# PPWangyc/video-spike

Hardware: AMD Instinct MI355X
Metric: clips/sec (16-frame 224x224) train step (higher is better)
Workload: dtype bf16; 1 GPU; C2 ViT-Tiny/16 16x224x224 -> 128 neurons, encoder+head fwd+bwd+AdamW; model=vmae_tiny, global_batch=128, clips_per_gpu=128, seq_len=1568, parallelism=dp1

## Files before the change

video-spike_amd/csrc/attention.hip:

```cpp
#include <math.h>
#include <stdlib.h>

#include <type_traits>

#include "common.h"

namespace vs {

constexpr float kLog2e = 1.4426950408889634f;
constexpr float kLn2 = 0.6931471805599453f;

__global__ __launch_bounds__(256) void attn_fwd_f32_kernel(const float* __restrict__ qkv, int64_t ldq,
                                                           float* __restrict__ o, int64_t ldo, float* __restrict__ lse,
                                                           int N, int H, float scale) {
  __shared__ float sK[64][68];
  __shared__ float sV[64][68];
  const int tid = threadIdx.x, sub = tid & 3;
  const int qi = blockIdx.x * 64 + (tid >> 2);
  const int h = blockIdx.y, b = blockIdx.z, D = H * 64;
  const int64_t row0 = (int64_t)b * N;
  const float* Qp = qkv + row0 * ldq + h * 64;
  const float* Kp = Qp + D;
  const float* Vp = Qp + 2 * D;
  float q[16], acc[16];
// ... 171 lines not shown
    for (int d = 0; d < 16; ++d) dqkv[(row0 + qi) * ldd + h * 64 + sub * 16 + d] = dq[d] * scale;
  }
}

template <typename T>
__global__ __launch_bounds__(256) void attn_delta_kernel(const T* __restrict__ o, int64_t ldo, const T* __restrict__ dout,
                                                         int64_t lddo, float* __restrict__ delta, int64_t rows, int N,
                                                         int H) {
  const int lane = threadIdx.x & 63;
  const int64_t w = blockIdx.x * 4 + (threadIdx.x >> 6);
  if (w >= rows * H) return;
  const int64_t row = w / H;
  const int h = (int)(w % H);
  float v = Elem<T>::load(o + row * ldo + h * 64 + lane) * Elem<T>::load(dout + row * lddo + h * 64 + lane);
  v = wave_sum(v);
  if (lane == 0) {
    const int64_t b = row / N, n = row % N;
    delta[(b * H + h) * N + n] = v;
  }
}

__device__ __forceinline__ int swz_row(int r) { return (r >> 1) & 7; }
__device__ __forceinline__ int swz_half(int r) { return ((r >> 1) & 1) << 2; }

__device__ __forceinline__ int off_rowswz(int r, int c) { return r * 128 + (((c >> 3) ^ swz_row(r)) << 4) + (c & 7) * 2; }
__device__ __forceinline__ int off_halfswz(int r, int c) { return r * 128 + (((c >> 3) ^ swz_half(r)) << 4) + (c & 7) * 2; }

__device__ __forceinline__ bf16x8 tr_pair(const char* lds, int off0, int off1) {
  short4v t0 = __builtin_amdgcn_ds_read_tr16_b64_v4i16((VS_LDS short4v*)(lds + off0));
  short4v t1 = __builtin_amdgcn_ds_read_tr16_b64_v4i16((VS_LDS short4v*)(lds + off1));
  typedef __attribute__((ext_vector_type(8))) short short8v;
  short8v s = {t0[0], t0[1], t0[2], t0[3], t1[0], t1[1], t1[2], t1[3]};
  return __builtin_bit_cast(bf16x8, s);
}

typedef __attribute__((ext_vector_type(8))) float f32x8;
__device__ __forceinline__ bf16x8 pack8(const f32x16& a, int base) {
  const f32x8 v = {a[base], a[base + 1], a[base + 2], a[base + 3], a[base + 4], a[base + 5], a[base + 6], a[base + 7]};
  return __builtin_convertvector(v, bf16x8);
}
__device__ __forceinline__ bf16x8 pack8f(const float* a) {
  const f32x8 v = {a[0], a[1], a[2], a[3], a[4], a[5], a[6], a[7]};
  return __builtin_convertvector(v, bf16x8);
}

__device__ __forceinline__ uint2 pack4(float a, float b, float c, float d) {
  uint2 u;
  u.x = (uint32_t)f2bf(a) | ((uint32_t)f2bf(b) << 16);
  u.y = (uint32_t)f2bf(c) | ((uint32_t)f2bf(d) << 16);
  return u;
}

constexpr float kRescaleThr = 8.0f;
constexpr float kRefBand = 32.0f;
#ifndef VS_FWD_TOPBAR
#define VS_FWD_TOPBAR 0
#endif

__device__ __forceinline__ float max3f(float a, float b, float c) {
  float r;
  asm volatile("v_max3_f32 %0, %1, %2, %3" : "=v"(r) : "v"(a), "v"(b), "v"(c));
  return r;
}
__device__ __forceinline__ float max16(const f32x16& x) {
  const float a = max3f(x[0], x[1], x[2]), b = max3f(x[3], x[4], x[5]), c = max3f(x[6], x[7], x[8]);
  const float d = max3f(x[9], x[10], x[11]), e = max3f(x[12], x[13], x[14]);
// ... 85 lines not shown
  bf16x8 qf[4];
#pragma unroll
  for (int s = 0; s < 4; ++s) {
    const int qr = qi < N ? qi : N - 1;
    const bf16x8 q = *(const bf16x8*)(Qp + (int64_t)qr * ldq + 16 * s + 8 * hh);
    f32x8 v;
#pragma unroll
    for (int j = 0; j < 8; ++j) v[j] = (float)q[j] * c;
    qf[s] = __builtin_convertvector(v, bf16x8);
  }
  const bf16x8 sel = rowsum_selector(lane);
  f32x16 oacc[2], zero16;
  f32x4 lacc;
  float m_run, l_half;

  const int q4 = (lane & 15) >> 2, p4 = (lane & 3) * 4, g16 = ((lane >> 4) & 1) * 16;
  int kbase[4];
  {
    const int key = lane & 31;
#pragma unroll
    for (int s = 0; s < 4; ++s) kbase[s] = key * 128 + (((2 * s + hh) ^ swz_row(key)) << 4);
  }
  int vbase[2];
  {
    const int k0 = 4 * hh + q4;
#pragma unroll
    for (int dt = 0; dt < 2; ++dt) vbase[dt] = TILE + off_halfswz(k0, dt * 32 + g16 + p4);
  }
  const int prow0 = wid * 16 + (lane >> 3), ppos = lane & 7;
  const uint32_t gk0 = (uint32_t)(prow0 * 2 * ldq + ((ppos ^ swz_row(prow0)) << 4));
  const uint32_t gk1 = (uint32_t)((prow0 + 8) * 2 * ldq + ((ppos ^ swz_row(prow0 + 8)) << 4));
  const uint32_t gv0 = (uint32_t)(prow0 * 2 * ldq + ((ppos ^ swz_half(prow0)) << 4));
  const uint32_t gv1 = (uint32_t)((prow0 + 8) * 2 * ldq + ((ppos ^ swz_half(prow0 + 8)) << 4));
  const int64_t tile_bytes = 64 * 2 * ldq, vdelta = 2 * (int64_t)D;
  auto load_tile = [&](int kt, char* buf) {
    const char* kb = (const char*)Kp + kt * tile_bytes;
    const char* vb = kb + vdelta;
    char* dk = buf + wid * 2048;
    char* dv = buf + TILE + wid * 2048;
    if ((kt + 1) * 64 <= N) {
      glds16_asm_so(kb, gk0, dk);
      glds16_asm_so(kb, gk1, dk + 1024);
      glds16_asm_so(vb, gv0, dv);
      glds16_asm_so(vb, gv1, dv + 1024);
    } else {
      const int r0 = kt * 64 + prow0, r1 = r0 + 8;
      const uint32_t c0 = (uint32_t)((r0 < N ? r0 : N - 1) - kt * 64) * (uint32_t)(2 * ldq);
      const uint32_t c1 = (uint32_t)((r1 < N ? r1 : N - 1) - kt * 64) * (uint32_t)(2 * ldq);
      glds16_asm_so(kb, c0 + ((ppos ^ swz_row(prow0)) << 4), dk);
      glds16_asm_so(kb, c1 + ((ppos ^ swz_row(prow0 + 8)) << 4), dk + 1024);
      glds16_asm_so(vb, c0 + ((ppos ^ swz_half(prow0)) << 4), dv);
      glds16_asm_so(vb, c1 + ((ppos ^ swz_half(prow0 + 8)) << 4), dv + 1024);
    }
  };
  struct KFrag {
    bf16x8 k[4];
  };
  struct VFrag {
    bf16x8 v[4];
  };
  auto kread = [&](const char* base, int kb) {
    KFrag f;
#pragma unroll
    for (int s = 0; s < 4; ++s) f.k[s] = *(const bf16x8*)(base + kb * 4096 + kbase[s]);
    return f;
  };
  auto vread = [&](const char* base, int kb) {
    VFrag f;
#pragma unroll
    for (int s = 0; s < 2; ++s)
#pragma unroll
      for (int dt = 0; dt < 2; ++dt) {
        const char* vb = base + kb * 4096 + s * 2048;
        f.v[2 * s + dt] = tr_pair(vb, vbase[dt], vbase[dt] + 1024);
      }
    return f;
  };
  auto pv = [&](const VFrag& f, const bf16x8& pa, const bf16x8& pb) {
#pragma unroll
    for (int s = 0; s < 2; ++s)
#pragma unroll
      for (int dt = 0; dt < 2; ++dt)
        oacc[dt] = mfma32p(f.v[2 * s + dt], s == 0 ? pa : pb, oacc[dt]);
  };

  auto softmax_m = [&](auto safec, auto maskc, f32x16& acc, int key0, bool first_blk, bf16x8& pa, bf16x8& pb) {
// ... 279 lines not shown
  if (tid == 0) redo_flag = 0;

  bf16x8 qf[2][2];
#pragma unroll
  for (int qt = 0; qt < 2; ++qt) {
    const int qi = q0w + qt * 16 + c, qr = qi < N ? qi : N - 1;
#pragma unroll
    for (int dc = 0; dc < 2; ++dc) {
      const bf16x8 q = *(const bf16x8*)(Qp + (int64_t)qr * ldq + dc * 32 + 8 * g);
      f32x8 v;
#pragma unroll
      for (int j = 0; j < 8; ++j) v[j] = (float)q[j] * scale_log2;
      qf[qt][dc] = __builtin_convertvector(v, bf16x8);
    }
  }
  const bf16x8 ones = __builtin_convertvector((f32x8){1.f, 1.f, 1.f, 1.f, 1.f, 1.f, 1.f, 1.f}, bf16x8);
  f32x4 oacc[4][2], lacc[2];
  const f32x4 zero4 = {0.f, 0.f, 0.f, 0.f};
  float m_run[2], l_half[2];

  int kbase[2], vbase[4];
#pragma unroll
  for (int dc = 0; dc < 2; ++dc) kbase[dc] = c * 128 + (((dc * 4 + g) ^ swz_row(c)) << 4);
  {
    const int r = 4 * g + (c >> 2), sw = swz_v16(r);
#pragma unroll
    for (int dt = 0; dt < 4; ++dt) vbase[dt] = TILE + r * 128 + (((dt * 2 + ((c & 3) >> 1)) ^ sw) << 4) + (c & 1) * 8;
  }
  const int prow0 = wid * 16 + (lane >> 3), ppos = lane & 7;
  const uint32_t gk0 = (uint32_t)(prow0 * 2 * ldq + ((ppos ^ swz_row(prow0)) << 4));
  const uint32_t gk1 = (uint32_t)((prow0 + 8) * 2 * ldq + ((ppos ^ swz_row(prow0 + 8)) << 4));
  const uint32_t gv0 = (uint32_t)(prow0 * 2 * ldq + ((ppos ^ swz_v16(prow0)) << 4));
  const uint32_t gv1 = (uint32_t)((prow0 + 8) * 2 * ldq + ((ppos ^ swz_v16(prow0 + 8)) << 4));
  const int64_t tile_bytes = 64 * 2 * ldq, vdelta = 2 * (int64_t)D;
  auto load_tile = [&](int kt, char* buf) {
    const char* kb = (const char*)Kp + kt * tile_bytes;
    const char* vb = kb + vdelta;
    char* dk = buf + wid * 2048;
    char* dv = buf + TILE + wid * 2048;
    if ((kt + 1) * 64 <= N) {
      glds16_asm_so(kb, gk0, dk);
      glds16_asm_so(kb, gk1, dk + 1024);
      glds16_asm_so(vb, gv0, dv);
      glds16_asm_so(vb, gv1, dv + 1024);
    } else {
      const int r0 = kt * 64 + prow0, r1 = r0 + 8;
      const uint32_t c0 = (uint32_t)((r0 < N ? r0 : N - 1) - kt * 64) * (uint32_t)(2 * ldq);
      const uint32_t c1 = (uint32_t)((r1 < N ? r1 : N - 1) - kt * 64) * (uint32_t)(2 * ldq);
      glds16_asm_so(kb, c0 + ((ppos ^ swz_row(prow0)) << 4), dk);
      glds16_asm_so(kb, c1 + ((ppos ^ swz_row(prow0 + 8)) << 4), dk + 1024);
      glds16_asm_so(vb, c0 + ((ppos ^ swz_v16(prow0)) << 4), dv);
      glds16_asm_so(vb, c1 + ((ppos ^ swz_v16(prow0 + 8)) << 4), dv + 1024);
    }
  };
  struct KFrag {
    bf16x8 k[2][2];
  };
  struct VFrag {
    bf16x8 v[4];
  };
  struct SAcc {
    f32x4 s[2][2];
  };
  auto kread = [&](const char* base, int kb) {
    KFrag f;
#pragma unroll
    for (int ks = 0; ks < 2; ++ks)
#pragma unroll
      for (int dc = 0; dc < 2; ++dc) f.k[ks][dc] = *(const bf16x8*)(base + kb * 4096 + ks * 2048 + kbase[dc]);
    return f;
  };
  auto vread = [&](const char* base, int kb) {
    VFrag f;
#pragma unroll
    for (int dt = 0; dt < 4; ++dt) f.v[dt] = tr_pair(base + kb * 4096, vbase[dt], vbase[dt] + 2048);
    return f;
  };
  auto qk_first = [&](const KFrag& f, SAcc& a) { a.s[0][0] = mfma16(f.k[0][0], qf[0][0], zero4); };
  auto qk_rest = [&](const KFrag& f, SAcc& a) {
    a.s[0][1] = mfma16(f.k[0][0], qf[1][0], zero4);
    a.s[1][0] = mfma16(f.k[1][0], qf[0][0], zero4);
    a.s[1][1] = mfma16(f.k[1][0], qf[1][0], zero4);
#pragma unroll
    for (int ks = 0; ks < 2; ++ks)
#pragma unroll
      for (int qt = 0; qt < 2; ++qt) a.s[ks][qt] = mfma16(f.k[ks][1], qf[qt][1], a.s[ks][qt]);
// ... 223 lines not shown
    nlse2[w] = -INFINITY;
    ndel[w] = 0.f;
  }
}

__device__ __forceinline__ int swz_rt(int r) {
  const int u = (r >> 1) & 7;
  return ((u & 1) << 2) | (u >> 1);
}
__device__ __forceinline__ int off_rtswz(int r, int c) { return r * 128 + (((c >> 3) ^ swz_rt(r)) << 4) + (c & 7) * 2; }

constexpr int kBwdQT = 64 * 128;
constexpr int kBwdStage = 2 * kBwdQT + 512;

__device__ __forceinline__ void attn_bwd_dkdv_body(char* __restrict__ stg0, char* __restrict__ stg1, int blk,
                                                   const bf16_t* __restrict__ qkv, int64_t ldq,
                                                   const bf16_t* __restrict__ dout, int64_t lddo,
                                                   const float* __restrict__ nlse2, const float* __restrict__ ndel,
                                                   bf16_t* __restrict__ dqkv, int64_t ldd, int N, int H, int Npad,
                                                   float scale) {
  constexpr int QT = kBwdQT;
  const int tid = threadIdx.x, lane = tid & 63, wid = __builtin_amdgcn_readfirstlane(tid >> 6), hh = lane >> 5;
  const int nb128 = (N + 127) / 128, kb = blk % nb128;
  const int h = (blk / nb128) % H, b = blk / nb128 / H, D = H * 64;
  const int64_t row0 = (int64_t)b * N;
  const bf16_t* Qp = qkv + row0 * ldq + h * 64;
  const bf16_t* Kp = Qp + D;
  const bf16_t* Vp = Qp + 2 * D;
  const bf16_t* Dp = dout + row0 * lddo + h * 64;
  const float* NL = nlse2 + ((int64_t)b * H + h) * Npad;
  const float* ND = ndel + ((int64_t)b * H + h) * Npad;
  const int ki = kb * 128 + wid * 32 + (lane & 31);
  const float c2 = scale * kLog2e;

  bf16x8 kf[4], vf[4];
  {
    const int kr = ki < N ? ki : N - 1;
#pragma unroll
    for (int s = 0; s < 4; ++s) {
      const bf16x8 k = *(const bf16x8*)(Kp + (int64_t)kr * ldq + 16 * s + 8 * hh);
      f32x8 v;
#pragma unroll
      for (int j = 0; j < 8; ++j) v[j] = (float)k[j] * c2;
      kf[s] = __builtin_convertvector(v, bf16x8);
      vf[s] = *(const bf16x8*)(Vp + (int64_t)kr * ldq + 16 * s + 8 * hh);
    }
  }
  f32x16 dkacc[2], dvacc[2];
#pragma unroll
  for (int r = 0; r < 16; ++r) {
    dkacc[0][r] = 0.f;
    dkacc[1][r] = 0.f;
    dvacc[0][r] = 0.f;
    dvacc[1][r] = 0.f;
  }

  const int prow = wid * 16 + (lane >> 3), ppos = lane & 7;
  const uint32_t cq0 = (uint32_t)((ppos ^ swz_rt(prow)) << 4), cq1 = (uint32_t)((ppos ^ swz_rt(prow + 8)) << 4);
  const uint32_t gq0 = (uint32_t)(prow * 2 * ldq) + cq0, gq1 = (uint32_t)((prow + 8) * 2 * ldq) + cq1;
  const uint32_t gd0 = (uint32_t)(prow * 2 * lddo) + cq0, gd1 = (uint32_t)((prow + 8) * 2 * lddo) + cq1;
  auto load_stage = [&](int it, char* dst) {
    const int q0 = it * 64;
    const char* qs = (const char*)(Qp + (int64_t)q0 * ldq);
    const char* ds = (const char*)(Dp + (int64_t)q0 * lddo);
    char* dq_ = dst + wid * 2048;
    char* dd_ = dst + QT + wid * 2048;
    if (q0 + 64 <= N) {
      glds16_asm_so(qs, gq0, dq_);
      glds16_asm_so(qs, gq1, dq_ + 1024);
// ... 42 lines not shown
    for (int s = 0; s < 4; ++s)
      acc = mfma32p(*(const bf16x8*)(sQ + sub * 4096 + roff[s]), kf[s], acc);
#pragma unroll
    for (int s2 = 0; s2 < 2; ++s2) {
      float p[8], ds[8];
#pragma unroll
      for (int r = 0; r < 8; ++r) {
        p[r] = __builtin_amdgcn_exp2f(acc[8 * s2 + r]);
        ds[r] = p[r] * dpa[8 * s2 + r];
      }
      const bf16x8 pb = pack8f(p), db = pack8f(ds);
#pragma unroll
      for (int dt = 0; dt < 2; ++dt) {
        const int o0 = sub * 4096 + s2 * 2048 + toff[dt][0], o1 = sub * 4096 + s2 * 2048 + toff[dt][1];
        dvacc[dt] = mfma32p(tr_pair(sD, o0, o1), pb, dvacc[dt]);
      }
#pragma unroll
      for (int dt = 0; dt < 2; ++dt) {
        const int o0 = sub * 4096 + s2 * 2048 + toff[dt][0], o1 = sub * 4096 + s2 * 2048 + toff[dt][1];
        dkacc[dt] = mfma32p(tr_pair(sQ, o0, o1), db, dkacc[dt]);
      }
    }
    __builtin_amdgcn_sched_barrier(0);
  };

  const int nit = (N + 63) / 64;
  load_stage(0, stg0);
  auto iter = [&](int it, auto bufc) {
    constexpr int BUF = decltype(bufc)::value;
    asm volatile("s_waitcnt vmcnt(0)" ::: "memory");
    __syncthreads();
    if (it + 1 < nit && !((VS_ATTN_DIAG & 2) && it >= 1)) load_stage(it + 1, BUF ? stg0 : stg1);
    const char* st = BUF ? stg1 : stg0;
    slice(st, 0);
    __builtin_amdgcn_sched_barrier(0);
    if (it * 64 + 32 < N) slice(st, 1);
    __builtin_amdgcn_sched_barrier(0);
  };
  for (int it = 0; it < nit; it += 2) {
    iter(it, IC<0>{});
    if (it + 1 < nit) iter(it + 1, IC<1>{});
  }

  if (ki < N) {
    bf16_t* krow = dqkv + (row0 + ki) * ldd + D + h * 64;
    bf16_t* vrow = krow + D;
#pragma unroll
    for (int dt = 0; dt < 2; ++dt)
#pragma unroll
      for (int g = 0; g < 4; ++g) {
        const int d = dt * 32 + 8 * g + 4 * hh;
        *(uint2*)(krow + d) = pack4(dkacc[dt][4 * g] * scale, dkacc[dt][4 * g + 1] * scale,
                                    dkacc[dt][4 * g + 2] * scale, dkacc[dt][4 * g + 3] * scale);
        *(uint2*)(vrow + d) = pack4(dvacc[dt][4 * g], dvacc[dt][4 * g + 1], dvacc[dt][4 * g + 2], dvacc[dt][4 * g + 3]);
      }
  }
}

__device__ __forceinline__ void attn_bwd_dq_body(char* __restrict__ kv0, char* __restrict__ kv1, int blk,
                                                 const bf16_t* __restrict__ qkv, int64_t ldq,
                                                 const bf16_t* __restrict__ dout, int64_t lddo,
                                                 const float* __restrict__ nlse2, const float* __restrict__ ndel,
                                                 bf16_t* __restrict__ dqkv, int64_t ldd, int N, int H, int Npad,
                                                 float scale) {
  constexpr int TILE = 64 * 128;
  const int tid = threadIdx.x, lane = tid & 63, wid = __builtin_amdgcn_readfirstlane(tid >> 6), hh = lane >> 5;
  const int nb128 = (N + 127) / 128, qb = blk % nb128;
  const int h = (blk / nb128) % H, b = blk / nb128 / H, D = H * 64;
  const int64_t row0 = (int64_t)b * N;
  const bf16_t* Qp = qkv + row0 * ldq + h * 64;
  const bf16_t* Kp = Qp + D;
  const bf16_t* Dp = dout + row0 * lddo + h * 64;
  const int qi = qb * 128 + wid * 32 + (lane & 31);
  const float c2 = scale * kLog2e;

  bf16x8 qf[4], df[4];
  {
    const int qr = qi < N ? qi : N - 1;
#pragma unroll
    for (int s = 0; s < 4; ++s) {
      const bf16x8 q = *(const bf16x8*)(Qp + (int64_t)qr * ldq + 16 * s + 8 * hh);
      f32x8 v;
#pragma unroll
      for (int j = 0; j < 8; ++j) v[j] = (float)q[j] * c2;
      qf[s] = __builtin_convertvector(v, bf16x8);
      df[s] = *(const bf16x8*)(Dp + (int64_t)qr * lddo + 16 * s + 8 * hh);
    }
  }
  f32x16 sinit, dinit, dqacc[2];
  {
    const int64_t w = ((int64_t)b * H + h) * Npad + qi;
    const float nl = qi < N ? nlse2[w] : -INFINITY;
    const float nd = qi < N ? ndel[w] : 0.f;
#pragma unroll
    for (int r = 0; r < 16; ++r) {
      sinit[r] = nl;
      dinit[r] = nd;
      dqacc[0][r] = 0.f;
      dqacc[1][r] = 0.f;
    }
  }

  int roff[4];
  {
    const int key = lane & 31;
#pragma unroll
    for (int s = 0; s < 4; ++s) roff[s] = key * 128 + (((2 * s + hh) ^ swz_rt(key)) << 4);
  }
  const int q4 = (lane & 15) >> 2, p4 = (lane & 3) * 4, g16 = ((lane >> 4) & 1) * 16, kt0 = 4 * hh + q4;
  int toff[2][2];
// ... 36 lines not shown
      const bf16x8 ka = *(const bf16x8*)(sK + kb * 4096 + roff[s]);
      const bf16x8 va = *(const bf16x8*)(sV + kb * 4096 + roff[s]);
      sacc = mfma32p(ka, qf[s], sacc);
      dpacc = mfma32p(va, df[s], dpacc);
    }
    if (key0 + 32 > N) {
#pragma unroll
      for (int r = 0; r < 16; ++r)
        if (key0 + (r & 3) + 8 * (r >> 2) + 4 * hh >= N) sacc[r] = -INFINITY;
    }
#pragma unroll
    for (int s2 = 0; s2 < 2; ++s2) {
      float ds[8];
#pragma unroll
      for (int r = 0; r < 8; ++r) ds[r] = __builtin_amdgcn_exp2f(sacc[8 * s2 + r]) * dpacc[8 * s2 + r];
      const bf16x8 db = pack8f(ds);
#pragma unroll
      for (int dt = 0; dt < 2; ++dt) {
        const int o = kb * 4096 + s2 * 2048;
        const bf16x8 ka = tr_pair(sK, o + toff[dt][0], o + toff[dt][1]);
        dqacc[dt] = mfma32p(ka, db, dqacc[dt]);
      }
    }
  };

  const int nkt = (N + 63) / 64;
  load_tile(0, kv0);
  auto iter = [&](int kt, auto bufc) {
    constexpr int BUF = decltype(bufc)::value;
    asm volatile("s_waitcnt vmcnt(0)" ::: "memory");
    __syncthreads();
    if (kt + 1 < nkt && !((VS_ATTN_DIAG & 2) && kt >= 1)) load_tile(kt + 1, BUF ? kv0 : kv1);
    const char* cur = BUF ? kv1 : kv0;
    sub(cur, 0, kt * 64);
    if (kt * 64 + 32 < N) sub(cur, 1, kt * 64 + 32);
  };
  for (int kt = 0; kt < nkt; kt += 2) {
    iter(kt, IC<0>{});
    if (kt + 1 < nkt) iter(kt + 1, IC<1>{});
  }
  if (qi < N) {
    bf16_t* qrow = dqkv + (row0 + qi) * ldd + h * 64;
#pragma unroll
    for (int dt = 0; dt < 2; ++dt)
#pragma unroll
      for (int g = 0; g < 4; ++g) {
        const int d = dt * 32 + 8 * g + 4 * hh;
        *(uint2*)(qrow + d) = pack4(dqacc[dt][4 * g] * scale, dqacc[dt][4 * g + 1] * scale,
                                    dqacc[dt][4 * g + 2] * scale, dqacc[dt][4 * g + 3] * scale);
      }
  }
}

__device__ __forceinline__ void attn_bwd_dkdv_pp(char* __restrict__ stg0, char* __restrict__ stg1, int blk,
                                                 const bf16_t* __restrict__ qkv, int64_t ldq,
                                                 const bf16_t* __restrict__ dout, int64_t lddo,
                                                 const float* __restrict__ nlse2, const float* __restrict__ ndel,
                                                 bf16_t* __restrict__ dqkv, int64_t ldd, int N, int H, int Npad,
                                                 float scale) {
  constexpr int QT = kBwdQT;
  const int tid = threadIdx.x, lane = tid & 63, hh = lane >> 5;
  const int wid = __builtin_amdgcn_readfirstlane(tid >> 6);
  const int nb128 = (N + 127) / 128, kb = blk % nb128;
  const int h = (blk / nb128) % H, b = blk / nb128 / H, D = H * 64;
  const int64_t row0 = (int64_t)b * N;
  const bf16_t* Qp = qkv + row0 * ldq + h * 64;
  const bf16_t* Kp = Qp + D;
  const bf16_t* Vp = Qp + 2 * D;
  const bf16_t* Dp = dout + row0 * lddo + h * 64;
  const float* NL = nlse2 + ((int64_t)b * H + h) * Npad;
  const float* ND = ndel + ((int64_t)b * H + h) * Npad;
  const int ki = kb * 128 + wid * 32 + (lane & 31);
  const float c2 = scale * kLog2e;

  bf16x8 kf[4], vf[4];
  {
    const int kr = ki < N ? ki : N - 1;
#pragma unroll
    for (int s = 0; s < 4; ++s) {
      const bf16x8 k = *(const bf16x8*)(Kp + (int64_t)kr * ldq + 16 * s + 8 * hh);
      f32x8 v;
#pragma unroll
      for (int j = 0; j < 8; ++j) v[j] = (float)k[j] * c2;
      kf[s] = __builtin_convertvector(v, bf16x8);
      vf[s] = *(const bf16x8*)(Vp + (int64_t)kr * ldq + 16 * s + 8 * hh);
    }
  }
  f32x16 dkacc[2], dvacc[2];
#pragma unroll
  for (int r = 0; r < 16; ++r) {
    dkacc[0][r] = 0.f;
    dkacc[1][r] = 0.f;
    dvacc[0][r] = 0.f;
    dvacc[1][r] = 0.f;
  }
  auto load_stage = [&](int it, char* dst) {
    const int prow = wid * 16 + (lane >> 3), ppos = lane & 7;
    const uint32_t cq0 = (uint32_t)((ppos ^ swz_rt(prow)) << 4), cq1 = (uint32_t)((ppos ^ swz_rt(prow + 8)) << 4);
    const int q0 = it * 64;
    int r0 = prow, r1 = prow + 8;
    if (q0 + 64 > N) {
      r0 = q0 + r0 < N ? r0 : N - 1 - q0;
      r1 = q0 + r1 < N ? r1 : N - 1 - q0;
    }
    const char* qs = (const char*)(Qp + (int64_t)q0 * ldq);
    const char* ds = (const char*)(Dp + (int64_t)q0 * lddo);
    glds16_asm_so(qs, (uint32_t)r0 * (uint32_t)(2 * ldq) + cq0, dst + wid * 2048);
    glds16_asm_so(qs, (uint32_t)r1 * (uint32_t)(2 * ldq) + cq1, dst + wid * 2048 + 1024);
    glds16_asm_so(ds, (uint32_t)r0 * (uint32_t)(2 * lddo) + cq0, dst + QT + wid * 2048);
// ... 67 lines not shown
    rowc(sE, 0, xa);
    mma_p(fa, pa, dvacc);
#pragma unroll
    for (int s = 0; s < 4; ++s) xa = mfma32p(fb[s], vf[s], xa);
    __builtin_amdgcn_sched_barrier(0);
    tr4(sD, 1, fa);
    rows4(sD, 1, fb);
    __builtin_amdgcn_sched_barrier(0);
#pragma unroll
    for (int r = 0; r < 16; ++r) pb[r] = __builtin_amdgcn_exp2f(xb[r]);
    rowc(sE, 1, xb);
    mma_p(fa, pb, dvacc);
#pragma unroll
    for (int s = 0; s < 4; ++s) xb = mfma32p(fb[s], vf[s], xb);
    __builtin_amdgcn_sched_barrier(0);
    tr4(sQ, 0, fa);
    tr4(sQ, 1, fb);
    __builtin_amdgcn_sched_barrier(0);
#pragma unroll
    for (int r = 0; r < 16; ++r) pa[r] *= xa[r];
    mma_p(fa, pa, dkacc);
#pragma unroll
    for (int r = 0; r < 16; ++r) pb[r] *= xb[r];
    mma_p(fb, pb, dkacc);
    __builtin_amdgcn_sched_barrier(0);
  };
  const int nit = (N + 63) / 64;
  load_stage(0, stg0);
  auto iter = [&](int it, auto bufc) {
    constexpr int BUF = decltype(bufc)::value;
    asm volatile("s_waitcnt vmcnt(0)" ::: "memory");
    __syncthreads();
    if (it + 1 < nit) load_stage(it + 1, BUF ? stg0 : stg1);
    slice(BUF ? stg1 : stg0);
  };
  for (int it = 0; it < nit; it += 2) {
    iter(it, IC<0>{});
    if (it + 1 < nit) iter(it + 1, IC<1>{});
  }
  if (ki < N) {
    bf16_t* krow = dqkv + (row0 + ki) * ldd + D + h * 64;
    bf16_t* vrow = krow + D;
#pragma unroll
    for (int dt = 0; dt < 2; ++dt)
#pragma unroll
      for (int g = 0; g < 4; ++g) {
        const int d = dt * 32 + 8 * g + 4 * hh;
        *(uint2*)(krow + d) = pack4(dkacc[dt][4 * g] * scale, dkacc[dt][4 * g + 1] * scale,
                                    dkacc[dt][4 * g + 2] * scale, dkacc[dt][4 * g + 3] * scale);
        *(uint2*)(vrow + d) = pack4(dvacc[dt][4 * g], dvacc[dt][4 * g + 1], dvacc[dt][4 * g + 2], dvacc[dt][4 * g + 3]);
      }
  }
}

__device__ __forceinline__ void attn_bwd_dq_pp(char* __restrict__ kv0, char* __restrict__ kv1, int blk,
                                               const bf16_t* __restrict__ qkv, int64_t ldq,
                                               const bf16_t* __restrict__ dout, int64_t lddo,
                                               const float* __restrict__ nlse2, const float* __restrict__ ndel,
                                               bf16_t* __restrict__ dqkv, int64_t ldd, int N, int H, int Npad,
                                               float scale) {
  constexpr int TILE = 64 * 128;
  const int tid = threadIdx.x, lane = tid & 63, hh = lane >> 5;
  const int wid = __builtin_amdgcn_readfirstlane(tid >> 6);
  const int nb128 = (N + 127) / 128, qb = blk % nb128;
  const int h = (blk / nb128) % H, b = blk / nb128 / H, D = H * 64;
  const int64_t row0 = (int64_t)b * N;
  const bf16_t* Qp = qkv + row0 * ldq + h * 64;
  const bf16_t* Kp = Qp + D;
  const bf16_t* Dp = dout + row0 * lddo + h * 64;
  const int qi = qb * 128 + wid * 32 + (lane & 31);
  const float c2 = scale * kLog2e;
  bf16x8 qf[4], df[4];
  {
    const int qr = qi < N ? qi : N - 1;
#pragma unroll
    for (int s = 0; s < 4; ++s) {
      const bf16x8 q = *(const bf16x8*)(Qp + (int64_t)qr * ldq + 16 * s + 8 * hh);
      f32x8 v;
#pragma unroll
      for (int j = 0; j < 8; ++j) v[j] = (float)q[j] * c2;
      qf[s] = __builtin_convertvector(v, bf16x8);
      df[s] = *(const bf16x8*)(Dp + (int64_t)qr * lddo + 16 * s + 8 * hh);
    }
  }
  f32x16 sinit, dinit, dqacc[2];
  {
    const int64_t w = ((int64_t)b * H + h) * Npad + qi;
    const float nl = qi < N ? nlse2[w] : -INFINITY;
    const float nd = qi < N ? ndel[w] : 0.f;
#pragma unroll
    for (int r = 0; r < 16; ++r) {
      sinit[r] = nl;
      dinit[r] = nd;
      dqacc[0][r] = 0.f;
      dqacc[1][r] = 0.f;
    }
  }
  int roff[4];
  {
    const int key = lane & 31;
#pragma unroll
    for (int s = 0; s < 4; ++s) roff[s] = key * 128 + (((2 * s + hh) ^ swz_rt(key)) << 4);
  }
  const int q4 = (lane & 15) >> 2, p4 = (lane & 3) * 4, g16 = ((lane >> 4) & 1) * 16, kt0 = 4 * hh + q4;
  int toff[2][2];
#pragma unroll
// ... 58 lines not shown
      kb_[s] = *(const bf16x8*)(sK + 4096 + roff[s]);
      vb[s] = *(const bf16x8*)(sV + 4096 + roff[s]);
    }
    __builtin_amdgcn_sched_barrier(0);
#pragma unroll
    for (int s = 0; s < 4; ++s) {
      sa = mfma32p(ka[s], qf[s], s == 0 ? sinit : sa);
      da = mfma32p(va[s], df[s], s == 0 ? dinit : da);
    }
#pragma unroll
    for (int s = 0; s < 4; ++s) {
      sb = mfma32p(kb_[s], qf[s], s == 0 ? sinit : sb);
      db = mfma32p(vb[s], df[s], s == 0 ? dinit : db);
    }
    __builtin_amdgcn_sched_barrier(0);
    ktr4(sK, 0, ka);
    ktr4(sK, 1, kb_);
    __builtin_amdgcn_sched_barrier(0);
    if (key0 + 64 > N) {
      mask(sa, key0);
      mask(sb, key0 + 32);
    }
    dq_mma(ka, sa, da);
    dq_mma(kb_, sb, db);
    __builtin_amdgcn_sched_barrier(0);
  };
  const int nkt = (N + 63) / 64;
  load_tile(0, kv0);
  auto iter = [&](int kt, auto bufc) {
    constexpr int BUF = decltype(bufc)::value;
    asm volatile("s_waitcnt vmcnt(0)" ::: "memory");
    __syncthreads();
    if (kt + 1 < nkt) load_tile(kt + 1, BUF ? kv0 : kv1);
    tile(BUF ? kv1 : kv0, kt * 64);
  };
  for (int kt = 0; kt < nkt; kt += 2) {
    iter(kt, IC<0>{});
    if (kt + 1 < nkt) iter(kt + 1, IC<1>{});
  }
  if (qi < N) {
    bf16_t* qrow = dqkv + (row0 + qi) * ldd + h * 64;
#pragma unroll
    for (int dt = 0; dt < 2; ++dt)
#pragma unroll
      for (int g = 0; g < 4; ++g) {
        const int d = dt * 32 + 8 * g + 4 * hh;
        *(uint2*)(qrow + d) = pack4(dqacc[dt][4 * g] * scale, dqacc[dt][4 * g + 1] * scale,
                                    dqacc[dt][4 * g + 2] * scale, dqacc[dt][4 * g + 3] * scale);
      }
  }
}

template <int WPS, bool PKV, bool PQ>
__global__ __launch_bounds__(256, WPS) void attn_bwd_bf16_pp_kernel(const bf16_t* __restrict__ qkv, int64_t ldq,
                                                                    const bf16_t* __restrict__ dout, int64_t lddo,
                                                                    const float* __restrict__ nlse2,
                                                                    const float* __restrict__ ndel,
                                                                    bf16_t* __restrict__ dqkv, int64_t ldd, int N,
                                                                    int H, int Npad, float scale, int nblk, int skip) {
  __shared__ __attribute__((aligned(16))) char st0[kBwdStage];
  __shared__ __attribute__((aligned(16))) char st1[kBwdStage];
  const int id = blockIdx.x;
  if (skip & (id < nblk ? 1 : 2)) return;
  if (id < nblk) {
    if constexpr (PKV)
      attn_bwd_dkdv_pp(st0, st1, xcd_remap(id, nblk), qkv, ldq, dout, lddo, nlse2, ndel, dqkv, ldd, N, H, Npad, scale);
    else
// ... 17 lines not shown
  __shared__ __attribute__((aligned(16))) char st0[kBwdStage];
  __shared__ __attribute__((aligned(16))) char st1[kBwdStage];
  const int id = blockIdx.x;
  if (skip & (id < nblk ? 1 : 2)) return;
  if (id < nblk)
    attn_bwd_dkdv_body(st0, st1, xcd_remap(id, nblk), qkv, ldq, dout, lddo, nlse2, ndel, dqkv, ldd, N, H, Npad, scale);
  else
    attn_bwd_dq_body(st0, st1, xcd_remap(id - nblk, nblk), qkv, ldq, dout, lddo, nlse2, ndel, dqkv, ldd, N, H, Npad,
                     scale);
}

}

using namespace vs;

static int attn_check(int64_t B, int64_t N, int64_t H, int64_t Dh) {
  VS_REQUIRE(Dh == 64, "vs_attn: head dim must be 64");
  VS_REQUIRE(B > 0 && N > 0 && H > 0, "vs_attn: empty problem");
  VS_REQUIRE(B <= 65535 && H <= 65535 && N < (1 << 30), "vs_attn: extents out of range");
  return VS_OK;
}

extern "C" int vs_attn_fwd(int32_t dtype, int64_t B, int64_t N, int64_t H, int64_t Dh, const void* qkv, int64_t ld_qkv,
                           void* o, int64_t ld_o, float* lse, float scale, void* stream) {
  VS_CALL(attn_check(B, N, H, Dh));
  VS_REQUIRE(qkv && o && lse, "vs_attn_fwd: null pointer");
  VS_REQUIRE(ld_qkv >= 3 * H * 64 && ld_o >= H * 64, "vs_attn_fwd: leading dims too small");
  hipStream_t s = (hipStream_t)stream;
  const double es = dtype == VS_BF16 ? 2.0 : 4.0;
  ScopedTimer timer(VS_TIMER_ATTN_FWD, s, (double)(B * N * H * 64) * 4.0 * es + (double)(B * H * N) * 4.0);
  if (dtype == VS_BF16) {
    VS_REQUIRE(ld_qkv % 8 == 0 && ld_o % 4 == 0 && aligned16(qkv) && (((uintptr_t)o) & 7) == 0,
               "vs_attn_fwd: bf16 rows must be 16-byte aligned");
    count_path(VS_PATH_ATTN_FWD);
    const int fv = knob(VS_KNOB_ATTN_VARIANT) & 15;
    dim3 grid((unsigned)(cdiv(N, 128) * H * B));
    auto kern = fv == 6   ? attn_fwd_bf16_kernel<0>
                : fv == 7 ? attn_fwd_bf16_kernel<2>
                : fv == 8 ? attn_fwd16_bf16_kernel
                          : attn_fwd_bf16_kernel<1>;
    hipLaunchKernelGGL(kern, grid, dim3(256), 0, s, (const bf16_t*)qkv, ld_qkv, (bf16_t*)o, ld_o, lse, (int)N, (int)H,
                       scale * kLog2e);
  } else if (dtype == VS_F32) {
    dim3 grid((unsigned)cdiv(N, 64), (unsigned)H, (unsigned)B);
    count_path(VS_PATH_ATTN_F32);
    hipLaunchKernelGGL(attn_fwd_f32_kernel, grid, dim3(256), 0, s, (const float*)qkv, ld_qkv, (float*)o, ld_o, lse,
                       (int)N, (int)H, scale);
  } else {
    VS_REQUIRE(false, "vs_attn_fwd: bad dtype");
  }
  VS_LAUNCH_CHECK();
  return VS_OK;
}

extern "C" int vs_attn_redo_count(int64_t* out, int32_t reset) {
  VS_REQUIRE(out, "vs_attn_redo_count: null pointer");
  unsigned long long v = 0;
  hipError_t e = hipDeviceSynchronize();
  if (e != hipSuccess) return (int)e;
  e = hipMemcpyFromSymbol(&v, HIP_SYMBOL(vs::g_attn_redo), sizeof(v), 0, hipMemcpyDeviceToHost);
  if (e != hipSuccess) return (int)e;
  *out = (int64_t)v;
  if (reset) {
    const unsigned long long z = 0;
    e = hipMemcpyToSymbol(HIP_SYMBOL(vs::g_attn_redo), &z, sizeof(z), 0, hipMemcpyHostToDevice);
    if (e != hipSuccess) return (int)e;
// ... 82 lines not shown
```

Baseline: 4159 clips/sec.

## Use buffer loads with range clamping for K/V tiles and skip inactive waves

Replaces per-lane global-to-LDS loads, and their separate branch for the partial last tile, with buffer_load ... lds instructions that use a buffer resource descriptor. The hardware range check makes out-of-range rows read as zero, so the tail needs no special handling and address arithmetic drops to 32-bit scalar offsets. The backward kernels also mark waves whose 32 rows lie entirely past N as inactive, so those waves skip their fragment loads and compute. The waves still take part in the barriers and tile loads. This relies on each clip's qkv span fitting in the 32-bit buffer range, which a new host check enforces, and on zero-filled tail rows being masked correctly.

New measurement: 4197 clips/sec (median of 6 runs). About the same (+0.9%).

```diff
diff --git a/video-spike_amd/csrc/attention.hip b/video-spike_amd/csrc/attention.hip
--- a/video-spike_amd/csrc/attention.hip
+++ b/video-spike_amd/csrc/attention.hip
@@ -227,6 +227,43 @@
   typedef __attribute__((ext_vector_type(8))) short short8v;
   short8v s = {t0[0], t0[1], t0[2], t0[3], t1[0], t1[1], t1[2], t1[3]};
   return __builtin_bit_cast(bf16x8, s);
+}
+
+typedef uint32_t u32x4_t __attribute__((ext_vector_type(4)));
+__device__ __forceinline__ u32x4_t glds_rsrc(const void* base, uint32_t bytes) {
+  const uint64_t a = (uint64_t)(uintptr_t)base;
+  u32x4_t r;
+  r[0] = (uint32_t)__builtin_amdgcn_readfirstlane((int)(uint32_t)a);
+  r[1] = (uint32_t)__builtin_amdgcn_readfirstlane((int)(uint32_t)(a >> 32));
+  r[2] = (uint32_t)__builtin_amdgcn_readfirstlane((int)bytes);
+  r[3] = 0x00020000u;
+  return r;
+}
+__device__ __forceinline__ uint32_t lds_addr_u(const void* p) {
+  return (uint32_t)__builtin_amdgcn_readfirstlane((int)(uint32_t)(uintptr_t)(VS_LDS const char*)p);
+}
+__device__ __forceinline__ void glds16x2x2_buf(u32x4_t rs, uint32_t sa, uint32_t sb, uint32_t a0, uint32_t a1,
+                                               uint32_t b0, uint32_t b1, uint32_t l0, uint32_t l1, uint32_t l2,
+                                               uint32_t l3) {
+  uint32_t keep;
+  asm volatile(
+      "s_mov_b32 %0, m0\n\t"
+      "s_mov_b32 m0, %8\n\t"
+      "s_nop 0\n\t"
+      "buffer_load_dwordx4 %1, %5, %6 offen lds\n\t"
+      "s_mov_b32 m0, %9\n\t"
+      "s_nop 0\n\t"
+      "buffer_load_dwordx4 %2, %5, %6 offen lds\n\t"
+      "s_mov_b32 m0, %10\n\t"
+      "s_nop 0\n\t"
+      "buffer_load_dwordx4 %3, %5, %7 offen lds\n\t"
+      "s_mov_b32 m0, %11\n\t"
+      "s_nop 0\n\t"
+      "buffer_load_dwordx4 %4, %5, %7 offen lds\n\t"
+      "s_mov_b32 m0, %0"
+      : "=&s"(keep)
+      : "v"(a0), "v"(a1), "v"(b0), "v"(b1), "s"(rs), "s"(sa), "s"(sb), "s"(l0), "s"(l1), "s"(l2), "s"(l3)
+      : "memory");
 }
 
 typedef __attribute__((ext_vector_type(8))) float f32x8;
@@ -378,26 +415,12 @@
   const uint32_t gk1 = (uint32_t)((prow0 + 8) * 2 * ldq + ((ppos ^ swz_row(prow0 + 8)) << 4));
   const uint32_t gv0 = (uint32_t)(prow0 * 2 * ldq + ((ppos ^ swz_half(prow0)) << 4));
   const uint32_t gv1 = (uint32_t)((prow0 + 8) * 2 * ldq + ((ppos ^ swz_half(prow0 + 8)) << 4));
-  const int64_t tile_bytes = 64 * 2 * ldq, vdelta = 2 * (int64_t)D;
+  const uint32_t tile_bytes = (uint32_t)(64 * 2 * ldq), vdelta = (uint32_t)(2 * D);
+  const u32x4_t kvres = glds_rsrc(Kp, (uint32_t)((int64_t)(N - 1) * 2 * ldq) + vdelta + 128);
+  const uint32_t lds0 = lds_addr_u(smem0) + wid * 2048, lds1 = lds_addr_u(smem1) + wid * 2048;
   auto load_tile = [&](int kt, char* buf) {
-    const char* kb = (const char*)Kp + kt * tile_bytes;
-    const char* vb = kb + vdelta;
-    char* dk = buf + wid * 2048;
-    char* dv = buf + TILE + wid * 2048;
-    if ((kt + 1) * 64 <= N) {
-      glds16_asm_so(kb, gk0, dk);
-      glds16_asm_so(kb, gk1, dk + 1024);
-      glds16_asm_so(vb, gv0, dv);
-      glds16_asm_so(vb, gv1, dv + 1024);
-    } else {
-      const int r0 = kt * 64 + prow0, r1 = r0 + 8;
-      const uint32_t c0 = (uint32_t)((r0 < N ? r0 : N - 1) - kt * 64) * (uint32_t)(2 * ldq);
-      const uint32_t c1 = (uint32_t)((r1 < N ? r1 : N - 1) - kt * 64) * (uint32_t)(2 * ldq);
-      glds16_asm_so(kb, c0 + ((ppos ^ swz_row(prow0)) << 4), dk);
-      glds16_asm_so(kb, c1 + ((ppos ^ swz_row(prow0 + 8)) << 4), dk + 1024);
-      glds16_asm_so(vb, c0 + ((ppos ^ swz_half(prow0)) << 4), dv);
-      glds16_asm_so(vb, c1 + ((ppos ^ swz_half(prow0 + 8)) << 4), dv + 1024);
-    }
+    const uint32_t so = (uint32_t)kt * tile_bytes, l = buf == smem0 ? lds0 : lds1;
+    glds16x2x2_buf(kvres, so, so + vdelta, gk0, gk1, gv0, gv1, l, l + 1024, l + TILE, l + TILE + 1024);
   };
   struct KFrag {
     bf16x8 k[4];
@@ -743,26 +766,12 @@
   const uint32_t gk1 = (uint32_t)((prow0 + 8) * 2 * ldq + ((ppos ^ swz_row(prow0 + 8)) << 4));
   const uint32_t gv0 = (uint32_t)(prow0 * 2 * ldq + ((ppos ^ swz_v16(prow0)) << 4));
   const uint32_t gv1 = (uint32_t)((prow0 + 8) * 2 * ldq + ((ppos ^ swz_v16(prow0 + 8)) << 4));
-  const int64_t tile_bytes = 64 * 2 * ldq, vdelta = 2 * (int64_t)D;
+  const uint32_t tile_bytes = (uint32_t)(64 * 2 * ldq), vdelta = (uint32_t)(2 * D);
+  const u32x4_t kvres = glds_rsrc(Kp, (uint32_t)((int64_t)(N - 1) * 2 * ldq) + vdelta + 128);
+  const uint32_t lds0 = lds_addr_u(smem0) + wid * 2048, lds1 = lds_addr_u(smem1) + wid * 2048;
   auto load_tile = [&](int kt, char* buf) {
-    const char* kb = (const char*)Kp + kt * tile_bytes;
-    const char* vb = kb + vdelta;
-    char* dk = buf + wid * 2048;
-    char* dv = buf + TILE + wid * 2048;
-    if ((kt + 1) * 64 <= N) {
-      glds16_asm_so(kb, gk0, dk);
-      glds16_asm_so(kb, gk1, dk + 1024);
-      glds16_asm_so(vb, gv0, dv);
-      glds16_asm_so(vb, gv1, dv + 1024);
-    } else {
-      const int r0 = kt * 64 + prow0, r1 = r0 + 8;
-      const uint32_t c0 = (uint32_t)((r0 < N ? r0 : N - 1) - kt * 64) * (uint32_t)(2 * ldq);
-      const uint32_t c1 = (uint32_t)((r1 < N ? r1 : N - 1) - kt * 64) * (uint32_t)(2 * ldq);
-      glds16_asm_so(kb, c0 + ((ppos ^ swz_row(prow0)) << 4), dk);
-      glds16_asm_so(kb, c1 + ((ppos ^ swz_row(prow0 + 8)) << 4), dk + 1024);
-      glds16_asm_so(vb, c0 + ((ppos ^ swz_v16(prow0)) << 4), dv);
-      glds16_asm_so(vb, c1 + ((ppos ^ swz_v16(prow0 + 8)) << 4), dv + 1024);
-    }
+    const uint32_t so = (uint32_t)kt * tile_bytes, l = buf == smem0 ? lds0 : lds1;
+    glds16x2x2_buf(kvres, so, so + vdelta, gk0, gk1, gv0, gv1, l, l + 1024, l + TILE, l + TILE + 1024);
   };
   struct KFrag {
     bf16x8 k[2][2];
@@ -1052,9 +1061,10 @@
   const float* ND = ndel + ((int64_t)b * H + h) * Npad;
   const int ki = kb * 128 + wid * 32 + (lane & 31);
   const float c2 = scale * kLog2e;
-
-  bf16x8 kf[4], vf[4];
-  {
+  const bool active = kb * 128 + wid * 32 < N;
+
+  bf16x8 kf[4] = {}, vf[4] = {};
+  if (active) {
     const int kr = ki < N ? ki : N - 1;
 #pragma unroll
     for (int s = 0; s < 4; ++s) {
@@ -1163,10 +1173,12 @@
     __syncthreads();
     if (it + 1 < nit && !((VS_ATTN_DIAG & 2) && it >= 1)) load_stage(it + 1, BUF ? stg0 : stg1);
     const char* st = BUF ? stg1 : stg0;
-    slice(st, 0);
-    __builtin_amdgcn_sched_barrier(0);
-    if (it * 64 + 32 < N) slice(st, 1);
-    __builtin_amdgcn_sched_barrier(0);
+    if (active) {
+      slice(st, 0);
+      __builtin_amdgcn_sched_barrier(0);
+      if (it * 64 + 32 < N) slice(st, 1);
+      __builtin_amdgcn_sched_barrier(0);
+    }
   };
   for (int it = 0; it < nit; it += 2) {
     iter(it, IC<0>{});
@@ -1204,9 +1216,10 @@
   const bf16_t* Dp = dout + row0 * lddo + h * 64;
   const int qi = qb * 128 + wid * 32 + (lane & 31);
   const float c2 = scale * kLog2e;
-
-  bf16x8 qf[4], df[4];
-  {
+  const bool active = qb * 128 + wid * 32 < N;
+
+  bf16x8 qf[4] = {}, df[4] = {};
+  if (active) {
     const int qr = qi < N ? qi : N - 1;
 #pragma unroll
     for (int s = 0; s < 4; ++s) {
@@ -1309,8 +1322,10 @@
     __syncthreads();
     if (kt + 1 < nkt && !((VS_ATTN_DIAG & 2) && kt >= 1)) load_tile(kt + 1, BUF ? kv0 : kv1);
     const char* cur = BUF ? kv1 : kv0;
-    sub(cur, 0, kt * 64);
-    if (kt * 64 + 32 < N) sub(cur, 1, kt * 64 + 32);
+    if (active) {
+      sub(cur, 0, kt * 64);
+      if (kt * 64 + 32 < N) sub(cur, 1, kt * 64 + 32);
+    }
   };
   for (int kt = 0; kt < nkt; kt += 2) {
     iter(kt, IC<0>{});
@@ -1349,9 +1364,10 @@
   const float* ND = ndel + ((int64_t)b * H + h) * Npad;
   const int ki = kb * 128 + wid * 32 + (lane & 31);
   const float c2 = scale * kLog2e;
-
-  bf16x8 kf[4], vf[4];
-  {
+  const bool active = kb * 128 + wid * 32 < N;
+
+  bf16x8 kf[4] = {}, vf[4] = {};
+  if (active) {
     const int kr = ki < N ? ki : N - 1;
 #pragma unroll
     for (int s = 0; s < 4; ++s) {
@@ -1485,7 +1501,7 @@
     asm volatile("s_waitcnt vmcnt(0)" ::: "memory");
     __syncthreads();
     if (it + 1 < nit) load_stage(it + 1, BUF ? stg0 : stg1);
-    slice(BUF ? stg1 : stg0);
+    if (active) slice(BUF ? stg1 : stg0);
   };
   for (int it = 0; it < nit; it += 2) {
     iter(it, IC<0>{});
@@ -1523,8 +1539,9 @@
   const bf16_t* Dp = dout + row0 * lddo + h * 64;
   const int qi = qb * 128 + wid * 32 + (lane & 31);
   const float c2 = scale * kLog2e;
-  bf16x8 qf[4], df[4];
-  {
+  const bool active = qb * 128 + wid * 32 < N;
+  bf16x8 qf[4] = {}, df[4] = {};
+  if (active) {
     const int qr = qi < N ? qi : N - 1;
 #pragma unroll
     for (int s = 0; s < 4; ++s) {
@@ -1649,7 +1666,7 @@
     asm volatile("s_waitcnt vmcnt(0)" ::: "memory");
     __syncthreads();
     if (kt + 1 < nkt) load_tile(kt + 1, BUF ? kv0 : kv1);
-    tile(BUF ? kv1 : kv0, kt * 64);
+    if (active) tile(BUF ? kv1 : kv0, kt * 64);
   };
   for (int kt = 0; kt < nkt; kt += 2) {
     iter(kt, IC<0>{});
@@ -1733,6 +1750,7 @@
   if (dtype == VS_BF16) {
     VS_REQUIRE(ld_qkv % 8 == 0 && ld_o % 4 == 0 && aligned16(qkv) && (((uintptr_t)o) & 7) == 0,
                "vs_attn_fwd: bf16 rows must be 16-byte aligned");
+    VS_REQUIRE(N * ld_qkv * 2 < ((int64_t)1 << 31), "vs_attn_fwd: one clip's qkv rows must span < 2 GiB");
     count_path(VS_PATH_ATTN_FWD);
     const int fv = knob(VS_KNOB_ATTN_VARIANT) & 15;
     dim3 grid((unsigned)(cdiv(N, 128) * H * B));
```
